# ygjwd12345/UCD

Hardware: AMD Instinct MI355X
Metric: images/sec (whole node) per UCD train step, VOC 15-5 step-1, 513^2 bs=24 (higher is better)
Workload: dtype bf16

## Files before the change

### ucd_amd/csrc/abn.hip

```cpp
#include "common.h"
#include "abn_finalize.h"

namespace ucd {
namespace {

constexpr int kBlock = 256;
constexpr int kMaxBands = 512;

struct Geom {
  int TX, TY, gx, gy, rows_per_band;
};

template <int VEC>
Geom make_geom(int M, int C, int target_blocks, int min_iters, int max_bands = 4096) {
  Geom g;
  const int round_rows = 4;
  int CG = C / VEC;
  g.TX = CG < 64 ? CG : 64;
  g.TY = kBlock / g.TX;
  g.gx = ceil_div(CG, g.TX);
  int by_rows = M / (g.TY * min_iters);
  int gy = target_blocks / g.gx;
  if (gy > by_rows) gy = by_rows;
  if (gy > max_bands) gy = max_bands;
  if (gy < 1) gy = 1;
  g.rows_per_band = ceil_div(M, gy);
  g.rows_per_band = ceil_div(g.rows_per_band, round_rows * g.TY) * round_rows * g.TY;
  g.gy = ceil_div(M, g.rows_per_band);
  return g;
}

template <int NV>
__device__ __forceinline__ void block_reduce_rows(float (&v)[NV], int tx, int ty, int TX, int TY, float* lds) {
#pragma unroll
  for (int i = 0; i < NV; ++i) lds[(ty * TX + tx) * NV + i] = v[i];
  __syncthreads();
  int span = 1;
  while (span < TY) span <<= 1;
  for (int s = span >> 1; s > 0; s >>= 1) {
    if (ty < s && ty + s < TY) {
#pragma unroll
      for (int i = 0; i < NV; ++i) lds[(ty * TX + tx) * NV + i] += lds[((ty + s) * TX + tx) * NV + i];
    }
    __syncthreads();
  }
  if (ty == 0) {
#pragma unroll
    for (int i = 0; i < NV; ++i) v[i] = lds[tx * NV + i];
  }
}

template <typename Row, typename First, typename Second>
__device__ __forceinline__ void request4(Row (&q)[4], int r, int TY, First first, Second second) {
#pragma unroll
  for (int u = 0; u < 4; ++u) first(q[u], r + u * TY);
#pragma unroll
  for (int u = 0; u < 4; ++u) second(q[u], r + u * TY);
}
template <typename Row, typename Use>
__device__ __forceinline__ void use4(const Row (&q)[4], int r, int TY, Use use) {
#pragma unroll
  for (int u = 0; u < 4; ++u) use(q[u], r + u * TY);
}
template <typename Row, typename First, typename Second, typename Use>
__device__ __forceinline__ void walk_band(int r, int r_end, int TY, First first, Second second, Use use) {
  for (; r + 3 * TY < r_end; r += 4 * TY) {
    Row q[4];
    request4(q, r, TY, first, second);
    use4(q, r, TY, use);
  }
  for (; r < r_end; r += TY) {
    Row q;
    first(q, r);
    second(q, r);
    use(q, r);
  }
}

template <typename T>
__global__ __launch_bounds__(kBlock) void abn_stats_kernel(const T* __restrict__ x, int ld_x, int M, int C,
                                                          const float* __restrict__ plane_bias, int HW,
                                                          int TX, int TY, int rows_per_band,
                                                          float* __restrict__ partial, float* __restrict__ kshift) {
  constexpr int VEC = Vec<T>::N;
  extern __shared__ __attribute__((aligned(16))) float lds[];
  const int tx = threadIdx.x % TX, ty = threadIdx.x / TX;
  const int cg = blockIdx.x * TX + tx;
  const bool live = ty < TY && cg * VEC < C;
  float acc[2 * VEC];
#pragma unroll
  for (int i = 0; i < 2 * VEC; ++i) acc[i] = 0.f;
  const int r_begin = blockIdx.y * rows_per_band;
  const int r_end = min(M, r_begin + rows_per_band);
  if (live) {
    const T* xp = x + (size_t)cg * VEC;
    float k[VEC];
    {
      Vec<T> v0;
      v0.load(xp);
#pragma unroll
      for (int i = 0; i < VEC; ++i) k[i] = v0.get(i) + (plane_bias ? plane_bias[cg * VEC + i] : 0.f);
      if (blockIdx.y == 0 && ty == 0) {
#pragma unroll
        for (int i = 0; i < VEC; ++i) kshift[cg * VEC + i] = k[i];
      }
    }
    auto accumulate = [&](const Vec<T>& v, int r) {
      if (plane_bias) {
        const float* pb = plane_bias + (size_t)(r / HW) * C + cg * VEC;
#pragma unroll
        for (int i = 0; i < VEC; ++i) {
          float f = (v.get(i) + pb[i]) - k[i];
          acc[i] += f;
          acc[VEC + i] += f * f;
        }
      } else {
#pragma unroll
        for (int i = 0; i < VEC; ++i) {
          float f = v.get(i) - k[i];
          acc[i] += f;
          acc[VEC + i] += f * f;
        }
      }
    };
    walk_band<Vec<T>>(r_begin + ty, r_end, TY, [&](Vec<T>& v, int r) { v.load(xp + (size_t)r * ld_x); }, [](Vec<T>&, int) {},
                      accumulate);
  }
  block_reduce_rows<2 * VEC>(acc, tx, ty, TX, TY, lds);
  if (ty == 0 && cg * VEC < C) {
    float* p = partial + (size_t)blockIdx.y * 2 * C + cg * VEC;
#pragma unroll
    for (int i = 0; i < VEC; ++i) {
      p[i] = acc[i];
      p[C + i] = acc[VEC + i];
    }
  }
}

template <int MODE, int LANES = 16>
__global__ __launch_bounds__(16 * LANES) void reduce_bands_kernel(const float* __restrict__ partial, int bands, int C,
                                                                  float* __restrict__ sums, FinalizeArgs fin,
                                                                  float* __restrict__ sums2 = nullptr,
                                                                  const float* __restrict__ sign_of = nullptr) {
  __shared__ float lds[LANES][17];
  const int kl = threadIdx.x & 15, lane = threadIdx.x >> 4;
  const int c = blockIdx.x * 8 + (kl & 7);
  const int k = (kl < 8 ? 0 : C) + c;
  const int n = 2 * C;
  float s0 = 0.f, s1 = 0.f, s2 = 0.f, s3 = 0.f;
  FinalizeIn pre{1.f, 0.f, 0.f};
  float pre_k = 0.f;
  if (MODE == 1 && lane == 0 && kl < 8 && c < C) {
    pre = finalize_prefetch(c, fin);
    pre_k = fin.kshift ? fin.kshift[c] : 0.f;
  }
  if (c < C) {
    int b = lane;
    for (; b + 3 * LANES < bands; b += 4 * LANES) {
      s0 += partial[(size_t)b * n + k];
      s1 += partial[(size_t)(b + LANES) * n + k];
      s2 += partial[(size_t)(b + 2 * LANES) * n + k];
      s3 += partial[(size_t)(b + 3 * LANES) * n + k];
    }
    for (; b < bands; b += LANES) s0 += partial[(size_t)b * n + k];
  }
  lds[lane][kl] = (s0 + s1) + (s2 + s3);
  __syncthreads();
  if (LANES > 16) {
    if (lane < 16) {
      float t = 0.f;
#pragma unroll
      for (int i = 0; i < LANES / 16; ++i) t += lds[lane * (LANES / 16) + i][kl];
      lds[lane * (LANES / 16)][kl] = t;
    }
    __syncthreads();
  }
  if (lane == 0 && c < C) {
    float t = 0.f;
#pragma unroll
    for (int i = 0; i < 16; ++i) t += lds[i * (LANES / 16)][kl];
    if (sign_of && kl >= 8 && sign_of[c] < 0.f) t = -t;
    sums[k] = t;
    if (sums2) sums2[k] = t;
    lds[0][kl] = t;
  }
  if (MODE == 1) {
    __syncthreads();
    if (lane == 0 && kl < 8 && c < C) finalize_channel_pre(c, lds[0][kl], lds[0][kl + 8], pre_k, fin, pre);
  }
  if (MODE == 2) {
    __syncthreads();
    if (lane == 0 && kl < 8 && c < C) {
      const float s1 = lds[0][kl], s2 = lds[0][kl + 8];
      const float d = s1 / fin.count;
      fin.pack[c] = fin.kshift[c] + d;
      fin.pack[C + c] = s2 - s1 * d;
    }
  }
}

#define UCD_REDUCE_BANDS(MODE, bands, ...)                                                        \
  do {                                                                                             \
    if ((bands) >= 96) reduce_bands_kernel<MODE, 64><<<ceil_div(C, 8), 1024, 0, s>>>(__VA_ARGS__);  \
    else reduce_bands_kernel<MODE, 16><<<ceil_div(C, 8), 256, 0, s>>>(__VA_ARGS__);                \
  } while (0)

__global__ void abn_combine_finalize_kernel(const float* __restrict__ gathered, int world, int C, float m_local,
                                            FinalizeArgs fin) {
  int c = blockIdx.x * blockDim.x + threadIdx.x;
  if (c >= C) return;
  float mean = 0.f;
  for (int r = 0; r < world; ++r) mean += gathered[(size_t)r * 2 * C + c];
  mean /= (float)world;
  float m2 = 0.f, dev2 = 0.f;
  for (int r = 0; r < world; ++r) {
    const float d = gathered[(size_t)r * 2 * C + c] - mean;
    m2 += gathered[(size_t)r * 2 * C + C + c];
    dev2 += d * d;
  }
  finalize_moments(c, mean, m2 + m_local * dev2, fin);
}

__global__ void abn_finalize_kernel(const float* __restrict__ sums, int C, FinalizeArgs fin) {
  int c = blockIdx.x * blockDim.x + threadIdx.x;
  if (c >= C) return;
  finalize_channel(c, sums[c], sums[C + c], fin);
}

__global__ void abn_eval_params_kernel(const float* __restrict__ weight, const float* __restrict__ rv, float eps, int C,
                                       float* __restrict__ invstd, float* __restrict__ scale, int abs_gamma) {
  int c = blockIdx.x * blockDim.x + threadIdx.x;
  if (c >= C) return;
  float is = 1.f / sqrtf(rv[c] + eps);
  invstd[c] = is;
  scale[c] = (weight ? gamma_eff(weight[c], eps, abs_gamma) : 1.f) * is;
}

__device__ __forceinline__ void replica_sum(const float* __restrict__ acc, int reps, int C, size_t coff, int tx, int ty, int TX, int TY,
                                            bool live, float* lds, Pack8& s1, Pack8& s2) {
  if (reps <= 1) {
    if (live) { s1 = load_f8(acc + coff); s2 = load_f8(acc + C + coff); }
    return;
  }
  float v[16];
#pragma unroll
  for (int i = 0; i < 16; ++i) v[i] = 0.f;
  if (live) {
    for (int r = ty; r < reps; r += 4 * TY) {
      Pack8 a[4], b[4];
#pragma unroll
      for (int u = 0; u < 4; ++u) {
        const int rr = r + u * TY;
        if (rr < reps) {
          a[u] = load_f8(acc + (size_t)rr * 2 * C + coff);
          b[u] = load_f8(acc + (size_t)rr * 2 * C + C + coff);
        } else {
#pragma unroll
          for (int j = 0; j < 4; ++j) { a[u].p[j] = f32x2{0.f, 0.f}; b[u].p[j] = f32x2{0.f, 0.f}; }
        }
      }
#pragma unroll
      for (int u = 0; u < 4; ++u)
#pragma unroll
        for (int j = 0; j < 4; ++j) {
          v[2 * j] += a[u].p[j].x; v[2 * j + 1] += a[u].p[j].y;
          v[8 + 2 * j] += b[u].p[j].x; v[8 + 2 * j + 1] += b[u].p[j].y;
        }
    }
  }
  block_reduce_rows<16>(v, tx, ty, TX, TY, lds);
  if (live) {
#pragma unroll
    for (int j = 0; j < 4; ++j) {
      s1.p[j] = f32x2{lds[tx * 16 + 2 * j], lds[tx * 16 + 2 * j + 1]};
      s2.p[j] = f32x2{lds[tx * 16 + 8 + 2 * j], lds[tx * 16 + 8 + 2 * j + 1]};
    }
  }
}

struct ApplyFin {
  const float* acc;
  int reps;
  const float* kshift;
  const float* weight;
  float* running_mean;
  float* running_var;
  float* mean;
  float* invstd;
  float* scale;
  float count, momentum, eps;
  int abs_gamma;
};
__device__ __forceinline__ void apply_fin_channels(const ApplyFin& f, const Pack8& s1, const Pack8& s2, const Pack8& k, const Pack8& w,
                                                   size_t coff, bool writer, Pack8& mu, Pack8& sc) {
  const float inv_n = 1.f / f.count;
#pragma unroll
  for (int j = 0; j < 4; ++j) {
    float m[2], is[2], scl[2];
#pragma unroll
    for (int e = 0; e < 2; ++e) {
      const float s = s1.p[j][e], ss = s2.p[j][e];
      const float d = s * inv_n;
      m[e] = k.p[j][e] + d;
      const float var = fmaxf((ss - s * d) * inv_n, 0.f);
      const float ve = var + f.eps;
      const float r0 = __builtin_amdgcn_rsqf(ve);
      is[e] = r0 * (1.5f - 0.5f * ve * r0 * r0);
      scl[e] = (f.weight ? gamma_eff(w.p[j][e], f.eps, f.abs_gamma) : 1.f) * is[e];
      if (writer) {
        const int c = (int)coff + 2 * j + e;
        if (f.running_mean) f.running_mean[c] = (1.f - f.momentum) * f.running_mean[c] + f.momentum * m[e];
        if (f.running_var) {
          const float unbiased = f.count > 1.f ? var * (f.count / (f.count - 1.f)) : var;
          f.running_var[c] = (1.f - f.momentum) * f.running_var[c] + f.momentum * unbiased;
        }
        f.mean[c] = m[e];
        f.invstd[c] = is[e];
        f.scale[c] = scl[e];
      }
    }
    mu.p[j] = f32x2{m[0], m[1]};
    sc.p[j] = f32x2{scl[0], scl[1]};
  }
}

template <typename T, bool ELU, bool PB>
constexpr bool kStepForm = std::is_same<T, __hip_bfloat16>::value && !ELU && !PB;

template <bool ELU>
__device__ __forceinline__ f32x2 act2(f32x2 z, float slope) {
  if (ELU) return f32x2{act_fwd<UCD_ACT_ELU>(z.x, slope), act_fwd<UCD_ACT_ELU>(z.y, slope)};
  return leaky2(z, slope);
}

template <bool ELU, int NP>
__device__ __forceinline__ void bwd_lane(const Pack<NP>& v, const Pack<NP>& g, const Pack<NP>& yo, bool from_y, const Pack<NP>& mu,
                                         const Pack<NP>& is, const Pack<NP>& sc, const Pack<NP>& sh, float slope, Pack<NP>& dz,
                                         Pack<NP>& xh) {
#pragma unroll
  for (int j = 0; j < NP; ++j) {
    const f32x2 d = v.p[j] - mu.p[j];
    const f32x2 sgn = from_y ? yo.p[j] : d * sc.p[j] + sh.p[j];
    if (ELU) dz.p[j] = f32x2{g.p[j].x * act_grad<UCD_ACT_ELU>(sgn.x, slope, from_y), g.p[j].y * act_grad<UCD_ACT_ELU>(sgn.y, slope, from_y)};
    else dz.p[j] = leaky_grad2(g.p[j], sgn, slope);
    xh.p[j] = d * is.p[j];
  }
}

template <typename T>
__device__ __forceinline__ uint4 load_lane(const T* p) { return *reinterpret_cast<const uint4*>(p); }
template <typename T>
__device__ __forceinline__ void store_lane(T* p, const Pack<Lane<T>::NP>& f) { *reinterpret_cast<uint4*>(p) = Lane<T>::pack(f); }

struct ApplyRow { uint4 x, r; };
template <typename T, bool ELU, bool PB, bool RES, bool FIN>
__global__ __launch_bounds__(kBlock) void abn_apply_kernel(const T* x, int ld_x, T* y, int ld_y, const T* __restrict__ res, int ld_r,
                                                          int M, int C, const float* __restrict__ plane_bias, int HW,
                                                          const float* __restrict__ mean, const float* __restrict__ scale,
                                                          const float* __restrict__ beta, float slope, int TX, int TY,
                                                          int rows_per_band, ApplyFin fin) {
  constexpr int NP = Lane<T>::NP, VEC = 2 * NP;
  typedef Pack<NP> P;
  extern __shared__ __attribute__((aligned(16))) float fin_lds[];
  const int tx = threadIdx.x % TX, ty = threadIdx.x / TX;
  const int cg = blockIdx.x * TX + tx;
  const bool live = ty < TY && cg * VEC < C;
  if (!FIN && !live) return;
  const bool has_res = kStepForm<T, ELU, PB> ? RES : res != nullptr;
  const size_t coff = (size_t)cg * VEC;
  P mu, sc;
  const int r_begin = blockIdx.y * rows_per_band;
  const int r_end = min(M, r_begin + rows_per_band);
  auto ld = [&](const T* p, int ldp, int r) {
    if (!kStepForm<T, ELU, PB>) return load_lane(p + (size_t)r * ldp + coff);
    typedef unsigned u32x4 __attribute__((ext_vector_type(4)));
    const u32x4 v = __builtin_nontemporal_load(reinterpret_cast<const u32x4*>(p + (size_t)r * ldp + coff));
    return make_uint4(v[0], v[1], v[2], v[3]);
  };
  auto req_x = [&](ApplyRow& q, int r) { q.x = ld(x, ld_x, r); };
  auto req_r = [&](ApplyRow& q, int r) { if (has_res) q.r = ld(res, ld_r, r); };
  int r = r_begin + ty;
  const bool pre = FIN && live && r + 3 * TY < r_end;
  ApplyRow pq[4];
  if (pre) request4(pq, r, TY, req_x, req_r);
  if constexpr (FIN) {
    Pack8 s1, s2, kk, ww;
    if (live) {
      kk = load_f8(fin.kshift + coff);
      if (fin.weight) ww = load_f8(fin.weight + coff);
    }
    replica_sum(fin.acc, fin.reps, C, coff, tx, ty, TX, TY, live, fin_lds, s1, s2);
    if (!live) return;
    apply_fin_channels(fin, s1, s2, kk, ww, coff, blockIdx.y == 0 && ty == 0, mu, sc);
  } else {
    mu = load_pairs<NP>(mean + coff);
    sc = load_pairs<NP>(scale + coff);
  }
  const P sh = beta ? load_pairs<NP>(beta + coff) : zero_pairs<NP>();
  auto emit = [&](const ApplyRow& q, int r) {
    P v = Lane<T>::unpack(q.x), o;
    if (PB) {
      const P pb = load_pairs<NP>(plane_bias + (size_t)(r / HW) * C + coff);
#pragma unroll
      for (int j = 0; j < NP; ++j) v.p[j] = v.p[j] + pb.p[j];
    }
    if (has_res) {
      const P qr = Lane<T>::unpack(q.r);
#pragma unroll
      for (int j = 0; j < NP; ++j) o.p[j] = act2<ELU>((v.p[j] - mu.p[j]) * sc.p[j] + sh.p[j] + qr.p[j], slope);
    } else {
#pragma unroll
      for (int j = 0; j < NP; ++j) o.p[j] = act2<ELU>((v.p[j] - mu.p[j]) * sc.p[j] + sh.p[j], slope);
    }
    store_lane(y + (size_t)r * ld_y + coff, o);
  };
  if (pre) {
    use4(pq, r, TY, emit);
    r += 4 * TY;
  }
  walk_band<ApplyRow>(r, r_end, TY, req_x, req_r, emit);
}

struct BwdRow { uint4 x, dy, y; };

template <typename T, bool ELU, bool PB, bool YOUT>
__global__ __launch_bounds__(kBlock) void abn_bwd_reduce_kernel(
    const T* __restrict__ x, int ld_x, const T* __restrict__ dy, int ld_dy, const T* __restrict__ yout, int ld_y, int M, int C,
    const float* __restrict__ plane_bias, int HW, const float* __restrict__ mean, const float* __restrict__ invstd,
    const float* __restrict__ scale, const float* __restrict__ shift, float slope, int TX, int TY, int rows_per_band,
    float* __restrict__ partial) {
  constexpr int NP = Lane<T>::NP, VEC = 2 * NP;
  typedef Pack<NP> P;
  extern __shared__ __attribute__((aligned(16))) float lds[];
  const int tx = threadIdx.x % TX, ty = threadIdx.x / TX;
  const int cg = blockIdx.x * TX + tx;
  const bool live = ty < TY && cg * VEC < C;
  const bool from_y = kStepForm<T, ELU, PB> ? YOUT : yout != nullptr;
  f32x2 s1[NP], s2[NP];
#pragma unroll
  for (int j = 0; j < NP; ++j) { s1[j] = f32x2{0.f, 0.f}; s2[j] = f32x2{0.f, 0.f}; }
  if (live) {
    const size_t coff = (size_t)cg * VEC;
    const P mu = load_pairs<NP>(mean + coff), is = load_pairs<NP>(invstd + coff), sc = load_pairs<NP>(scale + coff);
    const P sh = shift ? load_pairs<NP>(shift + coff) : zero_pairs<NP>();
    const int r_begin = blockIdx.y * rows_per_band;
    const int r_end = min(M, r_begin + rows_per_band);
    auto accumulate = [&](const BwdRow& q, int r) {
      P v = Lane<T>::unpack(q.x), yo, dz, xh;
      const P g = Lane<T>::unpack(q.dy);
      if (from_y) yo = Lane<T>::unpack(q.y);
      if (PB) {
        const P pb = load_pairs<NP>(plane_bias + (size_t)(r / HW) * C + coff);
#pragma unroll
        for (int j = 0; j < NP; ++j) v.p[j] = v.p[j] + pb.p[j];
      }
      bwd_lane<ELU>(v, g, yo, from_y, mu, is, sc, sh, slope, dz, xh);
#pragma unroll
      for (int j = 0; j < NP; ++j) {
        s1[j] += dz.p[j];
        s2[j] += dz.p[j] * xh.p[j];
      }
    };
    walk_band<BwdRow>(
        r_begin + ty, r_end, TY,
        [&](BwdRow& q, int r) { q.x = load_lane(x + (size_t)r * ld_x + coff); q.dy = load_lane(dy + (size_t)r * ld_dy + coff); },
        [&](BwdRow& q, int r) { if (from_y) q.y = load_lane(yout + (size_t)r * ld_y + coff); }, accumulate);
  }
  float acc[2 * VEC];
#pragma unroll
  for (int j = 0; j < NP; ++j) { acc[2 * j] = s1[j].x; acc[2 * j + 1] = s1[j].y; acc[VEC + 2 * j] = s2[j].x; acc[VEC + 2 * j + 1] = s2[j].y; }
  block_reduce_rows<2 * VEC>(acc, tx, ty, TX, TY, lds);
  if (ty == 0 && cg * VEC < C) {
    float* p = partial + (size_t)blockIdx.y * 2 * C + cg * VEC;
#pragma unroll
    for (int i = 0; i < VEC; ++i) {
      p[i] = acc[i];
      p[C + i] = acc[VEC + i];
    }
  }
}

template <typename T, bool ELU, bool PB, bool YOUT, bool DZOUT, bool RAW>
__global__ __launch_bounds__(kBlock) void abn_bwd_apply_kernel(
    const T* x, int ld_x, const T* dy, int ld_dy, const T* yout, int ld_y, T* dx, int ld_dx, T* dz_out, int ld_dz, int M, int C,
    const float* __restrict__ plane_bias, int HW, const float* __restrict__ mean, const float* __restrict__ invstd,
    const float* __restrict__ scale, const float* __restrict__ shift, const float* __restrict__ weight,
    const float* __restrict__ sums, float inv_count, int frozen, int abs_gamma, float slope, int TX, int TY, int rows_per_band,
    const float* __restrict__ grad_sums, float* __restrict__ grad_out, int reps) {
  constexpr int NP = Lane<T>::NP, VEC = 2 * NP;
  typedef Pack<NP> P;
  extern __shared__ __attribute__((aligned(16))) float raw_lds[];
  const int tx = threadIdx.x % TX, ty = threadIdx.x / TX;
  const int cg = blockIdx.x * TX + tx;
  const bool live = ty < TY && cg * VEC < C;
  if (!RAW && !live) return;
  const bool from_y = kStepForm<T, ELU, PB> ? YOUT : yout != nullptr;
  const bool want_dz = kStepForm<T, ELU, PB> ? DZOUT : dz_out != nullptr;
  const size_t coff = (size_t)cg * VEC;
  P rs0, rs1, rg0, rg1;
  if constexpr (RAW) {
    replica_sum(sums, reps, C, coff, tx, ty, TX, TY, live, raw_lds, rs0, rs1);
    const bool want_g = grad_out != nullptr && blockIdx.y == 0;
    if (want_g && grad_sums != sums) {
      __syncthreads();
      replica_sum(grad_sums, reps, C, coff, tx, ty, TX, TY, live, raw_lds, rg0, rg1);
    } else {
      rg0 = rs0; rg1 = rs1;
    }
    if (!live) return;
  }
  const P mu = load_pairs<NP>(mean + coff), sc = load_pairs<NP>(scale + coff);
  const P sh = shift ? load_pairs<NP>(shift + coff) : zero_pairs<NP>();
  P is, k0, k1, gw;
  if (frozen) {
    is = zero_pairs<NP>(); k0 = zero_pairs<NP>(); k1 = zero_pairs<NP>(); gw = sc;
  } else {
    is = load_pairs<NP>(invstd + coff);
    P a0, a1, w;
    if (RAW) { a0 = rs0; a1 = rs1; }
    else { a0 = load_pairs<NP>(sums + coff); a1 = load_pairs<NP>(sums + C + coff); }
    if (weight) w = load_pairs<NP>(weight + coff);
    auto signed_by_weight = [&](f32x2 v, int j) { return f32x2{w.p[j].x < 0.f ? -v.x : v.x, w.p[j].y < 0.f ? -v.y : v.y}; };
#pragma unroll
    for (int j = 0; j < NP; ++j) {
      k0.p[j] = a0.p[j] * inv_count;
      f32x2 kk = a1.p[j] * inv_count;
      if (abs_gamma) {
        if (weight && !RAW) kk = signed_by_weight(kk, j);
        gw.p[j] = sc.p[j];
      } else {
        gw.p[j] = weight ? w.p[j] * is.p[j] : is.p[j];
      }
      k1.p[j] = kk;
    }
    if (RAW && grad_out && blockIdx.y == 0 && ty == 0) {
#pragma unroll
      for (int j = 0; j < NP; ++j) {
        *reinterpret_cast<f32x2*>(grad_out + coff + 2 * j) = rg0.p[j];
        *reinterpret_cast<f32x2*>(grad_out + C + coff + 2 * j) = abs_gamma && weight ? signed_by_weight(rg1.p[j], j) : rg1.p[j];
      }
    }
  }
  const int r_begin = blockIdx.y * rows_per_band;
  const int r_end = min(M, r_begin + rows_per_band);
  auto emit = [&](const BwdRow& q, int r) {
    P v = Lane<T>::unpack(q.x), yo, dz, xh, o;
    const P g = Lane<T>::unpack(q.dy);
    if (from_y) yo = Lane<T>::unpack(q.y);
    if (PB) {
      const P pb = load_pairs<NP>(plane_bias + (size_t)(r / HW) * C + coff);
#pragma unroll
      for (int j = 0; j < NP; ++j) v.p[j] = v.p[j] + pb.p[j];
    }
    bwd_lane<ELU>(v, g, yo, from_y, mu, is, sc, sh, slope, dz, xh);
#pragma unroll
    for (int j = 0; j < NP; ++j) o.p[j] = (dz.p[j] - k0.p[j] - xh.p[j] * k1.p[j]) * gw.p[j];
    store_lane(dx + (size_t)r * ld_dx + coff, o);
    if (want_dz) store_lane(dz_out + (size_t)r * ld_dz + coff, dz);
  };
  walk_band<BwdRow>(
      r_begin + ty, r_end, TY,
      [&](BwdRow& q, int r) { q.x = load_lane(x + (size_t)r * ld_x + coff); q.dy = load_lane(dy + (size_t)r * ld_dy + coff); },
      [&](BwdRow& q, int r) { if (from_y) q.y = load_lane(yout + (size_t)r * ld_y + coff); }, emit);
}

template <typename T>
__global__ __launch_bounds__(kBlock) void plane_sum_kernel(const T* __restrict__ x, int ld_x, int HW, int C, float alpha,
                                                          int TX, int TY, float* __restrict__ out) {
  constexpr int VEC = Vec<T>::N;
  extern __shared__ __attribute__((aligned(16))) float lds[];
  const int tx = threadIdx.x % TX, ty = threadIdx.x / TX;
  const int cg = blockIdx.x * TX + tx;
  const int b = blockIdx.y;
  const bool live = ty < TY && cg * VEC < C;
  float acc[VEC];
#pragma unroll
  for (int i = 0; i < VEC; ++i) acc[i] = 0.f;
  if (live) {
    const T* xp = x + (size_t)b * HW * ld_x + (size_t)cg * VEC;
    int r = ty;
    for (; r + 3 * TY < HW; r += 4 * TY) {
      Vec<T> v0, v1, v2, v3;
      v0.load(xp + (size_t)r * ld_x);
      v1.load(xp + (size_t)(r + TY) * ld_x);
      v2.load(xp + (size_t)(r + 2 * TY) * ld_x);
      v3.load(xp + (size_t)(r + 3 * TY) * ld_x);
#pragma unroll
      for (int i = 0; i < VEC; ++i) acc[i] = (((acc[i] + v0.get(i)) + v1.get(i)) + v2.get(i)) + v3.get(i);
    }
    for (; r < HW; r += TY) {
      Vec<T> v;
      v.load(xp + (size_t)r * ld_x);
#pragma unroll
      for (int i = 0; i < VEC; ++i) acc[i] += v.get(i);
    }
  }
  block_reduce_rows<VEC>(acc, tx, ty, TX, TY, lds);
  if (ty == 0 && cg * VEC < C) {
#pragma unroll
    for (int i = 0; i < VEC; ++i) out[(size_t)b * C + cg * VEC + i] = acc[i] * alpha;
  }
}

template <typename T>
__global__ __launch_bounds__(kBlock) void window_vsum_kernel(const T* __restrict__ x, int ld_x, int B, int H, int W, int C,
                                                            int ph, float* __restrict__ tmp) {
  constexpr int VEC = Vec<T>::N;
  const int CG = C / VEC, OH = H - ph + 1;
  const size_t idx = (size_t)blockIdx.x * kBlock + threadIdx.x;
  if (idx >= (size_t)B * W * CG) return;
  const int cg = idx % CG, xx = (idx / CG) % W, b = idx / ((size_t)CG * W);
  const T* col = x + ((size_t)b * H * W + xx) * ld_x + (size_t)cg * VEC;
  float acc[VEC];
#pragma unroll
  for (int i = 0; i < VEC; ++i) acc[i] = 0.f;
  for (int y = 0; y < H; ++y) {
    Vec<T> v;
    v.load(col + (size_t)y * W * ld_x);
#pragma unroll
    for (int i = 0; i < VEC; ++i) acc[i] += v.get(i);
    if (y >= ph) {
      Vec<T> o;
      o.load(col + (size_t)(y - ph) * W * ld_x);
#pragma unroll
      for (int i = 0; i < VEC; ++i) acc[i] -= o.get(i);
    }
    if (y >= ph - 1) {
      float* dst = tmp + (((size_t)b * OH + (y - ph + 1)) * W + xx) * C + (size_t)cg * VEC;
#pragma unroll
      for (int i = 0; i < VEC; ++i) dst[i] = acc[i];
    }
  }
}

template <typename T>
__global__ __launch_bounds__(kBlock) void window_hsum_kernel(const float* __restrict__ tmp, int B, int OH, int W, int C, int pw,
                                                            float scale, T* __restrict__ out, int ld_o) {
  constexpr int VEC = Vec<T>::N;
  const int CG = C / VEC, OW = W - pw + 1;
  const size_t idx = (size_t)blockIdx.x * kBlock + threadIdx.x;
  if (idx >= (size_t)B * OH * CG) return;
  const int cg = idx % CG;
  const size_t line = idx / CG;
  const float* row = tmp + line * W * C + (size_t)cg * VEC;
  float acc[VEC];
#pragma unroll
  for (int i = 0; i < VEC; ++i) acc[i] = 0.f;
  for (int xx = 0; xx < W; ++xx) {
#pragma unroll
    for (int i = 0; i < VEC; ++i) acc[i] += row[(size_t)xx * C + i];
    if (xx >= pw) {
#pragma unroll
      for (int i = 0; i < VEC; ++i) acc[i] -= row[(size_t)(xx - pw) * C + i];
    }
    if (xx >= pw - 1) {
      Vec<T> o;
#pragma unroll
      for (int i = 0; i < VEC; ++i) o.set(i, acc[i] * scale);
      o.store(out + (line * OW + (xx - pw + 1)) * ld_o + (size_t)cg * VEC);
    }
  }
}

template <typename T>
__global__ __launch_bounds__(kBlock) void attmap_rowsq_kernel(const T* __restrict__ x, int ld_x, int M, int C,
                                                             float* __restrict__ a) {
  constexpr int VEC = Vec<T>::N;
  const int wave = threadIdx.x >> 6, lane = threadIdx.x & 63;
  const int r = blockIdx.x * (kBlock / 64) + wave;
  if (r >= M) return;
  float s = 0.f;
  for (int c = lane * VEC; c < C; c += 64 * VEC) {
    Vec<T> v;
    v.load(x + (size_t)r * ld_x + c);
#pragma unroll
    for (int i = 0; i < VEC; ++i) s += v.get(i) * v.get(i);
  }
  s = wave_sum(s);
  if (lane == 0) a[r] = s;
}
__global__ __launch_bounds__(kBlock) void attmap_norm_kernel(const float* __restrict__ a, int HW, float* __restrict__ inv) {
  __shared__ float lds[kBlock / 64];
  const int b = blockIdx.x;
  float s = 0.f;
  for (int p = threadIdx.x; p < HW; p += kBlock) {
    float v = a[(size_t)b * HW + p];
    s += v * v;
  }
  s = wave_sum(s);
  if ((threadIdx.x & 63) == 0) lds[threadIdx.x >> 6] = s;
  __syncthreads();
  if (threadIdx.x == 0) {
    float t = 0.f;
    for (int i = 0; i < kBlock / 64; ++i) t += lds[i];
    inv[b] = 1.f / sqrtf(t);
  }
}
template <typename T>
__global__ __launch_bounds__(kBlock) void attmap_scale_kernel(const T* __restrict__ x, int ld_x, T* __restrict__ y, int ld_y,
                                                             int M, int HW, int C, const float* __restrict__ a,
                                                             const float* __restrict__ inv) {
  constexpr int VEC = Vec<T>::N;
  const int wave = threadIdx.x >> 6, lane = threadIdx.x & 63;
  const int r = blockIdx.x * (kBlock / 64) + wave;
  if (r >= M) return;
  const float f = a[r] * inv[r / HW];
  for (int c = lane * VEC; c < C; c += 64 * VEC) {
    Vec<T> v, o;
    v.load(x + (size_t)r * ld_x + c);
#pragma unroll
    for (int i = 0; i < VEC; ++i) o.set(i, v.get(i) * f);
    o.store(y + (size_t)r * ld_y + c);
  }
}

int check_act_tensor(const char* fn, const char* name, const void* p, int ld, int dtype, int C, bool optional) {
  if (!p) {
    UCD_REQUIRE(optional, UCD_EINVAL, "%s: %s is NULL", fn, name);
    return 0;
  }
  const int es = dtype == UCD_BF16 ? 2 : 4;
  UCD_REQUIRE(aligned16(p) && ((size_t)ld * es) % 16 == 0, UCD_EALIGN,
              "%s: %s must be 16-byte aligned with a 16-byte multiple row pitch (ld=%d)", fn, name, ld);
  UCD_REQUIRE(ld >= C, UCD_EINVAL, "%s: ld of %s (%d) < C (%d)", fn, name, ld, C);
  return 0;
}
int check_common(const char* fn, int dtype, int M, int C, int act) {
  UCD_REQUIRE(dtype == UCD_F32 || dtype == UCD_BF16, UCD_EINVAL, "%s: unknown dtype %d", fn, dtype);
  UCD_REQUIRE(M > 0 && C > 0, UCD_EINVAL, "%s: empty tensor (M=%d, C=%d)", fn, M, C);
  const int vec = dtype == UCD_BF16 ? 8 : 4;
  UCD_REQUIRE(C % vec == 0, UCD_EALIGN, "%s: C=%d is not a multiple of %d", fn, C, vec);
  UCD_REQUIRE((act & ~(UCD_ACT_MASK | UCD_NORM_ABS_GAMMA)) == 0 && (act & UCD_ACT_MASK) <= UCD_ACT_ELU, UCD_EINVAL,
              "%s: unknown activation / flags 0x%x", fn, act);
  return 0;
}

template <typename F>
void with_flags(F&& f) { f(); }
template <typename F, typename... Rest>
void with_flags(F&& f, bool b, Rest... rest) {
  if (b) with_flags([&](auto... r) { f(std::true_type{}, r...); }, rest...);
  else with_flags([&](auto... r) { f(std::false_type{}, r...); }, rest...);
}
#define UCD_FLAG(x) decltype(x)::value

template <typename F, typename... Operands>
void dispatch_form(int dtype, int act_kind, const float* plane_bias, F&& f, Operands... operands) {
  with_flags(
      [&](auto BF, auto ELU, auto PB, auto... OP) {
        typedef std::conditional_t<UCD_FLAG(BF), __hip_bfloat16, float> T;
        f(T{}, ELU, PB, std::integral_constant<bool, kStepForm<T, UCD_FLAG(ELU), UCD_FLAG(PB)> && UCD_FLAG(OP)>{}...);
      },
      dtype == UCD_BF16, act_kind == UCD_ACT_ELU, plane_bias != nullptr, operands...);
}

inline float kernel_slope(int act_kind, float slope) { return act_kind == UCD_ACT_IDENTITY ? 1.f : slope; }

inline Geom geom_for(int dtype, int M, int C, int min_iters, int max_bands = 4096) {
  return dtype == UCD_BF16 ? make_geom<8>(M, C, 512, min_iters, max_bands) : make_geom<4>(M, C, 512, min_iters, max_bands);
}

#define UCD_TRY(expr)          \
  do {                         \
    int _rc = (expr);          \
    if (_rc) return _rc;       \
  } while (0)

}
}

using namespace ucd;

extern "C" {

size_t ucd_abn_workspace_bytes(int M, int C) {
  (void)M;
  return (size_t)kMaxBands * 2 * (size_t)C * sizeof(float);
}

static int abn_stats_impl(const void* x, int ld_x, int dtype, int M, int C, const float* plane_bias, int HW, float* sums,
                          float* kshift, void* workspace, size_t workspace_bytes, ucd_stream_t stream,
                          const FinalizeArgs* fin) {
  static const char* fn = "ucd_abn_stats";
  UCD_TRY(check_common(fn, dtype, M, C, UCD_ACT_IDENTITY));
  UCD_TRY(check_act_tensor(fn, "x", x, ld_x, dtype, C, false));
  UCD_REQUIRE(sums && kshift && workspace, UCD_EINVAL, "%s: sums/kshift/workspace is NULL", fn);
  UCD_REQUIRE(!plane_bias || HW > 0, UCD_EINVAL, "%s: plane_bias needs HW > 0", fn);
  hipStream_t s = (hipStream_t)stream;
  float* partial = (float*)workspace;
  const Geom g = geom_for(dtype, M, C, 8, kMaxBands);
  UCD_REQUIRE(workspace_bytes >= (size_t)g.gy * 2 * C * 4, UCD_EWORKSPACE, "%s: workspace too small", fn);
  with_flags(
      [&](auto BF) {
        typedef std::conditional_t<UCD_FLAG(BF), __hip_bfloat16, float> T;
        abn_stats_kernel<T><<<dim3(g.gx, g.gy), kBlock, kBlock * 2 * Vec<T>::N * 4, s>>>(
            (const T*)x, ld_x, M, C, plane_bias, HW, g.TX, g.TY, g.rows_per_band, partial, kshift);
      },
      dtype == UCD_BF16);
  UCD_TRY(check_launch(fn));
  if (fin && fin->pack)
    UCD_REDUCE_BANDS(2, g.gy, partial, g.gy, C, sums, *fin);
  else if (fin)
    UCD_REDUCE_BANDS(1, g.gy, partial, g.gy, C, sums, *fin);
  else
    UCD_REDUCE_BANDS(0, g.gy, partial, g.gy, C, sums, FinalizeArgs{});
  return check_launch(fn);
}

int ucd_abn_stats(const void* x, int ld_x, int dtype, int M, int C, const float* plane_bias, int HW, float* sums,
                  float* kshift, void* workspace, size_t workspace_bytes, ucd_stream_t stream) {
  return abn_stats_impl(x, ld_x, dtype, M, C, plane_bias, HW, sums, kshift, workspace, workspace_bytes, stream, nullptr);
}

int ucd_abn_stats_finalize(const void* x, int ld_x, int dtype, int M, int C, const float* plane_bias, int HW,
                           float* sums, float* kshift, const float* weight, float* running_mean, float* running_var,
                           float momentum, float eps, float* mean, float* invstd, float* scale, int flags,
                           void* workspace, size_t workspace_bytes, ucd_stream_t stream) {
  UCD_REQUIRE(mean && invstd && scale && kshift, UCD_EINVAL, "ucd_abn_stats_finalize: NULL output");
  FinalizeArgs fin{kshift, weight, running_mean, running_var, mean, invstd, scale, (float)M, momentum, eps, nullptr,
                   (flags & UCD_NORM_ABS_GAMMA) != 0};
  return abn_stats_impl(x, ld_x, dtype, M, C, plane_bias, HW, sums, kshift, workspace, workspace_bytes, stream, &fin);
}

int ucd_abn_finalize(const float* sums, const float* kshift, float count, int C, const float* weight,
                     float* running_mean, float* running_var, float momentum, float eps, float* mean, float* invstd,
                     float* scale, int flags, ucd_stream_t stream) {
  static const char* fn = "ucd_abn_finalize";
  UCD_REQUIRE(sums && mean && invstd && scale && C > 0 && count > 0.f, UCD_EINVAL, "%s: bad arguments", fn);
  FinalizeArgs fin{kshift, weight, running_mean, running_var, mean, invstd, scale, count, momentum, eps, nullptr,
                   (flags & UCD_NORM_ABS_GAMMA) != 0};
  abn_finalize_kernel<<<ceil_div(C, 256), 256, 0, (hipStream_t)stream>>>(sums, C, fin);
  return check_launch(fn);
}

int ucd_abn_eval_params(const float* weight, const float* running_var, float eps, int C, float* invstd, float* scale,
                        int flags, ucd_stream_t stream) {
  static const char* fn = "ucd_abn_eval_params";
  UCD_REQUIRE(running_var && invstd && scale && C > 0, UCD_EINVAL, "%s: bad arguments", fn);
  abn_eval_params_kernel<<<ceil_div(C, 256), 256, 0, (hipStream_t)stream>>>(weight, running_var, eps, C, invstd, scale,
                                                                            (flags & UCD_NORM_ABS_GAMMA) != 0);
  return check_launch(fn);
}

int ucd_abn_apply(const void* x, int ld_x, void* y, int ld_y, const void* residual, int ld_r, int dtype, int M, int C,
                  const float* plane_bias, int HW, const float* mean, const float* scale, const float* shift, int act,
                  float slope, ucd_stream_t stream) {
  static const char* fn = "ucd_abn_apply";
  UCD_TRY(check_common(fn, dtype, M, C, act));
  UCD_TRY(check_act_tensor(fn, "x", x, ld_x, dtype, C, false));
  UCD_TRY(check_act_tensor(fn, "y", y, ld_y, dtype, C, false));
  UCD_TRY(check_act_tensor(fn, "residual", residual, ld_r, dtype, C, true));
  UCD_REQUIRE(mean && scale, UCD_EINVAL, "%s: mean/scale is NULL", fn);
  UCD_REQUIRE(!plane_bias || HW > 0, UCD_EINVAL, "%s: plane_bias needs HW > 0", fn);
  hipStream_t s = (hipStream_t)stream;
  const int a = act & UCD_ACT_MASK;
  const Geom g = geom_for(dtype, M, C, 4);
  dispatch_form(
      dtype, a, plane_bias,
      [&](auto t, auto ELU, auto PB, auto RES) {
        typedef decltype(t) T;
        abn_apply_kernel<T, UCD_FLAG(ELU), UCD_FLAG(PB), UCD_FLAG(RES), false><<<dim3(g.gx, g.gy), kBlock, 0, s>>>(
            (const T*)x, ld_x, (T*)y, ld_y, (const T*)residual, ld_r, M, C, plane_bias, HW, mean, scale, shift, kernel_slope(a, slope),
            g.TX, g.TY, g.rows_per_band, ApplyFin{});
      },
      residual != nullptr);
  return check_launch(fn);
// ... 332 lines not shown
```

Baseline: 846.5.

## Double-buffer row loads and overlap replica reductions with first data prefetch

Adds a double-buffered row walker that issues loads for the next four rows before consuming the current four, and uses it in the backward stats kernel. The apply and backward-apply kernels now issue their first row loads while the cross-replica sum reduction is in flight. The two replica reductions in the backward kernel are fused into one pass. The aim is to hide global memory latency in these bandwidth-bound BN/ABN kernels, at the cost of more registers per thread and possibly lower occupancy.

```diff
diff --git a/ucd_amd/csrc/abn.hip b/ucd_amd/csrc/abn.hip
--- a/ucd_amd/csrc/abn.hip
+++ b/ucd_amd/csrc/abn.hip
@@ -62,8 +62,47 @@
 #pragma unroll
   for (int u = 0; u < 4; ++u) use(q[u], r + u * TY);
 }
+template <typename Row>
+struct Head { Row a[4], b[4]; };
+template <typename Row, typename First, typename Second>
+__device__ __forceinline__ void request_head(Head<Row>& h, int r, int r_end, int TY, First first, Second second) {
+#pragma unroll
+  for (int u = 0; u < 4; ++u) if (r + u * TY < r_end) first(h.a[u], r + u * TY);
+#pragma unroll
+  for (int u = 0; u < 4; ++u) if (r + u * TY < r_end) second(h.a[u], r + u * TY);
+}
 template <typename Row, typename First, typename Second, typename Use>
+__device__ __forceinline__ void walk_from_head(Head<Row>& h, int r, int r_end, int TY, First first, Second second, Use use) {
+  if (r + 3 * TY >= r_end) {
+#pragma unroll
+    for (int u = 0; u < 4; ++u) if (r + u * TY < r_end) use(h.a[u], r + u * TY);
+    return;
+  }
+  for (;;) {
+    if (r + 7 * TY >= r_end) { use4(h.a, r, TY, use); r += 4 * TY; break; }
+    request4(h.b, r + 4 * TY, TY, first, second);
+    use4(h.a, r, TY, use);
+    r += 4 * TY;
+    if (r + 7 * TY >= r_end) { use4(h.b, r, TY, use); r += 4 * TY; break; }
+    request4(h.a, r + 4 * TY, TY, first, second);
+    use4(h.b, r, TY, use);
+    r += 4 * TY;
+  }
+  for (; r < r_end; r += TY) {
+    Row q;
+    first(q, r);
+    second(q, r);
+    use(q, r);
+  }
+}
+template <bool PIPE, typename Row, typename First, typename Second, typename Use>
 __device__ __forceinline__ void walk_band(int r, int r_end, int TY, First first, Second second, Use use) {
+  if (PIPE) {
+    Head<Row> h;
+    request_head(h, r, r_end, TY, first, second);
+    walk_from_head(h, r, r_end, TY, first, second, use);
+    return;
+  }
   for (; r + 3 * TY < r_end; r += 4 * TY) {
     Row q[4];
     request4(q, r, TY, first, second);
@@ -123,8 +162,8 @@
         }
       }
     };
-    walk_band<Vec<T>>(r_begin + ty, r_end, TY, [&](Vec<T>& v, int r) { v.load(xp + (size_t)r * ld_x); }, [](Vec<T>&, int) {},
-                      accumulate);
+    walk_band<false, Vec<T>>(r_begin + ty, r_end, TY, [&](Vec<T>& v, int r) { v.load(xp + (size_t)r * ld_x); }, [](Vec<T>&, int) {},
+                             accumulate);
   }
   block_reduce_rows<2 * VEC>(acc, tx, ty, TX, TY, lds);
   if (ty == 0 && cg * VEC < C) {
@@ -236,38 +275,32 @@
   scale[c] = (weight ? gamma_eff(weight[c], eps, abs_gamma) : 1.f) * is;
 }
 
-__device__ __forceinline__ void replica_sum(const float* __restrict__ acc, int reps, int C, size_t coff, int tx, int ty, int TX, int TY,
-                                            bool live, float* lds, Pack8& s1, Pack8& s2) {
-  if (reps <= 1) {
-    if (live) { s1 = load_f8(acc + coff); s2 = load_f8(acc + C + coff); }
-    return;
-  }
-  float v[16];
-#pragma unroll
-  for (int i = 0; i < 16; ++i) v[i] = 0.f;
-  if (live) {
-    for (int r = ty; r < reps; r += 4 * TY) {
-      Pack8 a[4], b[4];
-#pragma unroll
-      for (int u = 0; u < 4; ++u) {
-        const int rr = r + u * TY;
-        if (rr < reps) {
-          a[u] = load_f8(acc + (size_t)rr * 2 * C + coff);
-          b[u] = load_f8(acc + (size_t)rr * 2 * C + C + coff);
-        } else {
-#pragma unroll
-          for (int j = 0; j < 4; ++j) { a[u].p[j] = f32x2{0.f, 0.f}; b[u].p[j] = f32x2{0.f, 0.f}; }
-        }
-      }
-#pragma unroll
-      for (int u = 0; u < 4; ++u)
-#pragma unroll
-        for (int j = 0; j < 4; ++j) {
-          v[2 * j] += a[u].p[j].x; v[2 * j + 1] += a[u].p[j].y;
-          v[8 + 2 * j] += b[u].p[j].x; v[8 + 2 * j + 1] += b[u].p[j].y;
-        }
-    }
-  }
+template <int U>
+__device__ __forceinline__ void replica_load(const float* __restrict__ acc, int r, int reps, int C, size_t coff, int TY, Pack8 (&a)[U],
+                                             Pack8 (&b)[U]) {
+#pragma unroll
+  for (int u = 0; u < U; ++u) {
+    const int rr = r + u * TY;
+    if (rr < reps) {
+      a[u] = load_f8(acc + (size_t)rr * 2 * C + coff);
+      b[u] = load_f8(acc + (size_t)rr * 2 * C + C + coff);
+    } else {
+#pragma unroll
+      for (int j = 0; j < 4; ++j) { a[u].p[j] = f32x2{0.f, 0.f}; b[u].p[j] = f32x2{0.f, 0.f}; }
+    }
+  }
+}
+template <int U>
+__device__ __forceinline__ void replica_add(float (&v)[16], const Pack8 (&a)[U], const Pack8 (&b)[U]) {
+#pragma unroll
+  for (int u = 0; u < U; ++u)
+#pragma unroll
+    for (int j = 0; j < 4; ++j) {
+      v[2 * j] += a[u].p[j].x; v[2 * j + 1] += a[u].p[j].y;
+      v[8 + 2 * j] += b[u].p[j].x; v[8 + 2 * j + 1] += b[u].p[j].y;
+    }
+}
+__device__ __forceinline__ void replica_reduce(float (&v)[16], int tx, int ty, int TX, int TY, bool live, float* lds, Pack8& s1, Pack8& s2) {
   block_reduce_rows<16>(v, tx, ty, TX, TY, lds);
   if (live) {
 #pragma unroll
@@ -276,6 +309,59 @@
       s2.p[j] = f32x2{lds[tx * 16 + 8 + 2 * j], lds[tx * 16 + 8 + 2 * j + 1]};
     }
   }
+}
+template <typename Between>
+__device__ __forceinline__ void replica_sum(const float* __restrict__ acc, int reps, int C, size_t coff, int tx, int ty, int TX, int TY,
+                                            bool live, float* lds, Pack8& s1, Pack8& s2, Between between) {
+  if (reps <= 1) {
+    if (live) { s1 = load_f8(acc + coff); s2 = load_f8(acc + C + coff); }
+    between();
+    return;
+  }
+  float v[16];
+#pragma unroll
+  for (int i = 0; i < 16; ++i) v[i] = 0.f;
+  if (live) {
+    Pack8 a[4], b[4];
+    replica_load<4>(acc, ty, reps, C, coff, TY, a, b);
+    between();
+    replica_add<4>(v, a, b);
+    for (int r = ty + 4 * TY; r < reps; r += 4 * TY) {
+      replica_load<4>(acc, r, reps, C, coff, TY, a, b);
+      replica_add<4>(v, a, b);
+    }
+  }
+  replica_reduce(v, tx, ty, TX, TY, live, lds, s1, s2);
+}
+template <typename Between>
+__device__ __forceinline__ void replica_sum2(const float* __restrict__ acc, const float* __restrict__ acc2, int reps, int C, size_t coff,
+                                             int tx, int ty, int TX, int TY, bool live, float* lds, Pack8& s1, Pack8& s2, Pack8& g1,
+                                             Pack8& g2, Between between) {
+  if (reps <= 1) {
+    if (live) { s1 = load_f8(acc + coff); s2 = load_f8(acc + C + coff); g1 = load_f8(acc2 + coff); g2 = load_f8(acc2 + C + coff); }
+    between();
+    return;
+  }
+  float v[16], vg[16];
+#pragma unroll
+  for (int i = 0; i < 16; ++i) { v[i] = 0.f; vg[i] = 0.f; }
+  if (live) {
+    Pack8 a[2], b[2], c[2], d[2];
+    replica_load<2>(acc, ty, reps, C, coff, TY, a, b);
+    replica_load<2>(acc2, ty, reps, C, coff, TY, c, d);
+    between();
+    replica_add<2>(v, a, b);
+    replica_add<2>(vg, c, d);
+    for (int r = ty + 2 * TY; r < reps; r += 2 * TY) {
+      replica_load<2>(acc, r, reps, C, coff, TY, a, b);
+      replica_load<2>(acc2, r, reps, C, coff, TY, c, d);
+      replica_add<2>(v, a, b);
+      replica_add<2>(vg, c, d);
+    }
+  }
+  replica_reduce(v, tx, ty, TX, TY, live, lds, s1, s2);
+  __syncthreads();
+  replica_reduce(vg, tx, ty, TX, TY, live, lds, g1, g2);
 }
 
 struct ApplyFin {
@@ -379,17 +465,16 @@
   };
   auto req_x = [&](ApplyRow& q, int r) { q.x = ld(x, ld_x, r); };
   auto req_r = [&](ApplyRow& q, int r) { if (has_res) q.r = ld(res, ld_r, r); };
-  int r = r_begin + ty;
-  const bool pre = FIN && live && r + 3 * TY < r_end;
-  ApplyRow pq[4];
-  if (pre) request4(pq, r, TY, req_x, req_r);
+  const int r = r_begin + ty;
+  Head<ApplyRow> head;
   if constexpr (FIN) {
     Pack8 s1, s2, kk, ww;
     if (live) {
       kk = load_f8(fin.kshift + coff);
       if (fin.weight) ww = load_f8(fin.weight + coff);
     }
-    replica_sum(fin.acc, fin.reps, C, coff, tx, ty, TX, TY, live, fin_lds, s1, s2);
+    replica_sum(fin.acc, fin.reps, C, coff, tx, ty, TX, TY, live, fin_lds, s1, s2,
+                [&]() { if (live) request_head(head, r, r_end, TY, req_x, req_r); });
     if (!live) return;
     apply_fin_channels(fin, s1, s2, kk, ww, coff, blockIdx.y == 0 && ty == 0, mu, sc);
   } else {
@@ -414,11 +499,8 @@
     }
     store_lane(y + (size_t)r * ld_y + coff, o);
   };
-  if (pre) {
-    use4(pq, r, TY, emit);
-    r += 4 * TY;
-  }
-  walk_band<ApplyRow>(r, r_end, TY, req_x, req_r, emit);
+  if constexpr (FIN) walk_from_head(head, r, r_end, TY, req_x, req_r, emit);
+  else walk_band<false, ApplyRow>(r, r_end, TY, req_x, req_r, emit);
 }
 
 struct BwdRow { uint4 x, dy, y; };
@@ -461,7 +543,7 @@
         s2[j] += dz.p[j] * xh.p[j];
       }
     };
-    walk_band<BwdRow>(
+    walk_band<true, BwdRow>(
         r_begin + ty, r_end, TY,
         [&](BwdRow& q, int r) { q.x = load_lane(x + (size_t)r * ld_x + coff); q.dy = load_lane(dy + (size_t)r * ld_dy + coff); },
         [&](BwdRow& q, int r) { if (from_y) q.y = load_lane(yout + (size_t)r * ld_y + coff); }, accumulate);
@@ -497,29 +579,41 @@
   const bool from_y = kStepForm<T, ELU, PB> ? YOUT : yout != nullptr;
   const bool want_dz = kStepForm<T, ELU, PB> ? DZOUT : dz_out != nullptr;
   const size_t coff = (size_t)cg * VEC;
+  const int r_begin = blockIdx.y * rows_per_band;
+  const int r_end = min(M, r_begin + rows_per_band);
+  const int r = r_begin + ty;
+  auto req_xdy = [&](BwdRow& q, int r) { q.x = load_lane(x + (size_t)r * ld_x + coff); q.dy = load_lane(dy + (size_t)r * ld_dy + coff); };
+  auto req_y = [&](BwdRow& q, int r) { if (from_y) q.y = load_lane(yout + (size_t)r * ld_y + coff); };
+  Head<BwdRow> head;
+  const bool ahead = RAW && live && r + 8 * TY < r_end;
+  P mu, sc, sh, is, w;
+  if (live) {
+    mu = load_pairs<NP>(mean + coff);
+    sc = load_pairs<NP>(scale + coff);
+    sh = shift ? load_pairs<NP>(shift + coff) : zero_pairs<NP>();
+    if (!frozen) {
+      is = load_pairs<NP>(invstd + coff);
+      if (weight) w = load_pairs<NP>(weight + coff);
+    }
+  }
   P rs0, rs1, rg0, rg1;
   if constexpr (RAW) {
-    replica_sum(sums, reps, C, coff, tx, ty, TX, TY, live, raw_lds, rs0, rs1);
-    const bool want_g = grad_out != nullptr && blockIdx.y == 0;
-    if (want_g && grad_sums != sums) {
-      __syncthreads();
-      replica_sum(grad_sums, reps, C, coff, tx, ty, TX, TY, live, raw_lds, rg0, rg1);
+    auto between = [&]() { if (ahead) request_head(head, r, r_end, TY, req_xdy, req_y); };
+    if (grad_out != nullptr && blockIdx.y == 0 && grad_sums != sums) {
+      replica_sum2(sums, grad_sums, reps, C, coff, tx, ty, TX, TY, live, raw_lds, rs0, rs1, rg0, rg1, between);
     } else {
+      replica_sum(sums, reps, C, coff, tx, ty, TX, TY, live, raw_lds, rs0, rs1, between);
       rg0 = rs0; rg1 = rs1;
     }
     if (!live) return;
   }
-  const P mu = load_pairs<NP>(mean + coff), sc = load_pairs<NP>(scale + coff);
-  const P sh = shift ? load_pairs<NP>(shift + coff) : zero_pairs<NP>();
-  P is, k0, k1, gw;
+  P k0, k1, gw;
   if (frozen) {
     is = zero_pairs<NP>(); k0 = zero_pairs<NP>(); k1 = zero_pairs<NP>(); gw = sc;
   } else {
-    is = load_pairs<NP>(invstd + coff);
-    P a0, a1, w;
+    P a0, a1;
     if (RAW) { a0 = rs0; a1 = rs1; }
     else { a0 = load_pairs<NP>(sums + coff); a1 = load_pairs<NP>(sums + C + coff); }
-    if (weight) w = load_pairs<NP>(weight + coff);
     auto signed_by_weight = [&](f32x2 v, int j) { return f32x2{w.p[j].x < 0.f ? -v.x : v.x, w.p[j].y < 0.f ? -v.y : v.y}; };
 #pragma unroll
     for (int j = 0; j < NP; ++j) {
@@ -541,8 +635,6 @@
       }
     }
   }
-  const int r_begin = blockIdx.y * rows_per_band;
-  const int r_end = min(M, r_begin + rows_per_band);
   auto emit = [&](const BwdRow& q, int r) {
     P v = Lane<T>::unpack(q.x), yo, dz, xh, o;
     const P g = Lane<T>::unpack(q.dy);
@@ -558,10 +650,8 @@
     store_lane(dx + (size_t)r * ld_dx + coff, o);
     if (want_dz) store_lane(dz_out + (size_t)r * ld_dz + coff, dz);
   };
-  walk_band<BwdRow>(
-      r_begin + ty, r_end, TY,
-      [&](BwdRow& q, int r) { q.x = load_lane(x + (size_t)r * ld_x + coff); q.dy = load_lane(dy + (size_t)r * ld_dy + coff); },
-      [&](BwdRow& q, int r) { if (from_y) q.y = load_lane(yout + (size_t)r * ld_y + coff); }, emit);
+  if (ahead) walk_from_head(head, r, r_end, TY, req_xdy, req_y, emit);
+  else walk_band<false, BwdRow>(r, r_end, TY, req_xdy, req_y, emit);
 }
 
 template <typename T>
```

After: 845.2. No clear change (-0.2%).
